# manoskary/analysisgnn

Measured on AMD Instinct MI355X. Metric: subgraph-nodes/sec fwd+bwd, HybridGNN L=3 H=256, higher is better.
Workload: dtype f32; 1 GPU; C2 (sampled, the batch a training step sees): HybridGNN L=3 H=256 out=128, 21 task heads, 32 neighbour-sampled subgraphs x (500 target notes + [5,5] hops) per GPU, per-hop counts passed (every layer trimmed); 16335 notes, 104099 edges per GPU; train step = fwd + objective (wloss) + bwd + allreduce + clip + AdamW, CSR rebuilt every step; hipGraph replay; workload_id=c2s, per_gpu_subgraphs=32, objective=wloss, parallelism=dp1, allreduce=none (one rank)

## Files before the change

analysisgnn_amd/_lib.py:

```python
from __future__ import annotations

import ctypes as C
import os
from typing import Optional, Sequence

import torch

_HERE = os.path.dirname(os.path.abspath(__file__))
LIB_PATH = os.path.join(_HERE, "libagnn_hip.so")
MAX_SEG = 32

SPMM_MEAN, SPMM_SKIP_SELF, SPMM_ACCUM = 1, 2, 4
INT32_MAX = 2 ** 31 - 1


class AgnnError(RuntimeError):
    pass


class CooSeg(C.Structure):
    _fields_ = [("row", C.c_void_p), ("col", C.c_void_p), ("etype", C.c_void_p),
                ("etype_code", C.c_int64), ("n_edges", C.c_int64), ("n_rows", C.c_int64)]


# ... 67 lines not shown
    _fields_ = [("dst", C.c_void_p), ("src", C.c_void_p * PACK_MAX_SRC), ("ld_dst", C.c_int64), ("ld_src", C.c_int64),
                ("rows", C.c_int32), ("cols", C.c_int32), ("n_src", C.c_int32), ("vec_ok", C.c_int32)]


_lib: Optional[C.CDLL] = None

SIGNATURES = {
    "agnn_last_error": (C.c_char_p, []),
    "agnn_version": (C.c_int, []),
    "agnn_csr_workspace_bytes": (C.c_size_t, [C.c_int64, C.c_int64]),
    "agnn_csr_build": (C.c_int, [C.c_int, C.POINTER(CooSeg), C.c_void_p, C.c_void_p, C.c_void_p,
                                 C.c_void_p, C.c_size_t, C.c_void_p, C.c_void_p]),
    "agnn_check_status": (C.c_int, [C.c_void_p, C.c_void_p]),
    "agnn_csr_rowend": (C.c_int, [C.c_void_p, C.c_void_p, C.c_int64, C.c_int64, C.c_void_p, C.c_void_p]),
    "agnn_csr_rowend_batch": (C.c_int, [C.c_int, C.POINTER(RowendItem), C.c_void_p]),
    "agnn_spmm_f32": (C.c_int, [C.c_int, C.POINTER(Rel), C.c_int64, C.c_int32, C.c_void_p, C.c_int64,
                                C.c_int64, C.c_void_p, C.c_int64, C.c_void_p, C.c_int32, C.c_uint32,
                                C.c_void_p]),
    "agnn_spmm_root_f32": (C.c_int, [C.c_int, C.POINTER(Rel), C.c_int64, C.c_int32, C.c_void_p, C.c_int64,
                                     C.c_int64, C.c_void_p, C.c_int64, C.c_int64, C.c_void_p, C.c_int32, C.c_uint32,
                                     C.c_void_p]),
    "agnn_gru_fwd_f32": (C.c_int, [C.c_void_p, C.c_void_p, C.c_void_p, C.c_int64, C.c_int64, C.c_int32,
                                   C.c_void_p, C.c_void_p, C.c_void_p, C.c_void_p, C.c_void_p]),
    "agnn_gru_bwd_f32": (C.c_int, [C.c_void_p, C.c_void_p, C.c_void_p, C.c_void_p, C.c_int64, C.c_int64,
                                   C.c_int32, C.c_void_p, C.c_void_p, C.c_void_p, C.c_void_p, C.c_void_p]),
    "agnn_heads_fwd_f32": (C.c_int, [C.c_void_p, C.c_int64, C.c_int64, C.c_int32, C.c_int32, C.c_int32, C.c_void_p, C.c_void_p,
                                     C.c_void_p, C.c_void_p, C.c_float, C.c_void_p, C.c_void_p, C.c_void_p, C.POINTER(C.c_int32),
                                     C.c_void_p, C.c_void_p, C.c_int64, C.c_void_p, C.c_void_p, C.c_void_p, C.c_int64, C.c_void_p]),
    "agnn_gru_hprev_f32": (C.c_int, [C.c_void_p, C.c_int64, C.c_int64, C.c_int32, C.c_void_p, C.c_void_p]),
    "agnn_hgt_attn_fwd_multi_f32": (C.c_int, [C.c_int32, C.c_void_p, C.c_int32, C.c_int32, C.c_void_p]),
    "agnn_hgt_attn_fwd_f32": (C.c_int, [C.c_int, C.POINTER(HgtRel), C.c_void_p, C.c_int64, C.c_int64, C.c_int32,
                                        C.c_int32, C.c_void_p, C.c_int64, C.c_void_p, C.c_void_p, C.c_void_p]),
    "agnn_hgt_attn_bwd_dst_f32": (C.c_int, [C.c_int, C.POINTER(HgtRel), C.c_void_p, C.c_int64, C.c_void_p, C.c_int64,
                                            C.c_void_p, C.c_int64, C.c_void_p, C.c_void_p, C.c_int64, C.c_int32,
                                            C.c_int32, C.c_void_p, C.c_int64, C.c_void_p]),
    "agnn_hgt_attn_bwd_src_batch_f32": (C.c_int, [C.c_int32, C.POINTER(HgtSrcItem), C.c_void_p, C.c_int64, C.c_void_p, C.c_int64,
                                                  C.c_int32, C.c_int32, C.c_void_p]),
    "agnn_sampler_num_nodes": (C.c_int64, [C.POINTER(Sampler)]),
    "agnn_sampler_edge_capacity": (C.c_int64, [C.POINTER(Sampler)]),
    "agnn_sample_hops": (C.c_int, [C.POINTER(Sampler), C.c_void_p]),
    "agnn_sample_members": (C.c_int, [C.c_void_p, C.c_int64, C.c_void_p, C.c_void_p, C.c_void_p, C.c_int32, C.c_int32, C.c_int32,
                                      C.POINTER(C.c_int32), C.c_int32, C.c_void_p, C.c_void_p, C.c_void_p, C.c_void_p]),
    "agnn_sample_compact_nodes": (C.c_int64, [C.POINTER(Sampler), C.POINTER(C.c_int32)]),
    "agnn_sample_compact": (C.c_int, [C.POINTER(Sampler), C.POINTER(C.c_int32), C.c_void_p, C.c_void_p, C.c_void_p]),
    "agnn_gather_rows_f32": (C.c_int, [C.c_void_p, C.c_int64, C.c_void_p, C.c_int64, C.c_int32, C.c_void_p, C.c_int64, C.c_void_p]),
    "agnn_gather_i64": (C.c_int, [C.c_void_p, C.c_int64, C.c_void_p, C.c_int64, C.c_int32, C.c_int64, C.c_void_p, C.c_int64, C.c_void_p]),
    "agnn_relt_fwd_f32": (C.c_int, [C.c_int, C.POINTER(ReltItem), C.c_int32, C.c_int32, C.c_int32, C.c_int64, C.c_void_p]),
    "agnn_relt_bwd_f32": (C.c_int, [C.c_int, C.POINTER(ReltItem), C.c_int32, C.c_int32, C.c_int32, C.c_int64, C.c_void_p]),
    "agnn_relt_dw_workspace_bytes": (C.c_size_t, [C.c_int, C.c_int32, C.c_int32, C.c_int32, C.c_int64]),
    "agnn_relt_dw_f32": (C.c_int, [C.c_int, C.POINTER(ReltItem), C.c_int32, C.c_int32, C.c_int32, C.c_int64, C.c_void_p, C.c_size_t,
                                  C.c_void_p]),
    "agnn_wgrad_batch_workspace_bytes": (C.c_size_t, [C.c_int32, C.POINTER(WgradItem)]),
    "agnn_wgrad_batch_f32": (C.c_int, [C.c_int32, C.POINTER(WgradItem), C.c_void_p, C.c_size_t, C.c_void_p]),
    "agnn_gemm_nt_f32": (C.c_int, [C.c_void_p, C.c_int64, C.c_void_p, C.c_int64, C.c_void_p, C.c_int64, C.c_int32, C.c_int32, C.c_void_p,
                                   C.c_int64, C.c_void_p]),
    "agnn_gemm_nn_f32": (C.c_int, [C.c_void_p, C.c_int64, C.c_void_p, C.c_int64, C.c_void_p, C.c_int64, C.c_int32, C.c_int32, C.c_void_p,
                                   C.c_int64, C.c_void_p]),
    "agnn_absdiff_fwd_f32": (C.c_int, [C.c_void_p, C.c_void_p, C.c_void_p, C.c_int64, C.c_int64, C.c_int32, C.c_void_p, C.c_void_p, C.c_int64,
                                       C.c_void_p]),
    "agnn_absdiff_bwd_f32": (C.c_int, [C.c_void_p, C.c_void_p, C.c_void_p, C.c_int64, C.c_int64, C.c_int32, C.c_void_p, C.c_void_p, C.c_int64,
                                       C.c_int32, C.c_int32, C.c_void_p, C.c_int64, C.c_void_p]),
    "agnn_gated_fwd_f32": (C.c_int, [C.POINTER(Gated), C.c_void_p, C.c_int64, C.c_void_p]),
    "agnn_gated_bwd_dst_f32": (C.c_int, [C.POINTER(Gated), C.c_void_p, C.c_int64, C.c_void_p, C.c_void_p, C.c_void_p]),
    "agnn_gated_bwd_src_f32": (C.c_int, [C.POINTER(Gated), C.c_void_p, C.c_int64, C.c_void_p, C.c_void_p, C.c_void_p]),
    "agnn_norm_act_workspace_bytes": (C.c_size_t, [C.c_int32]),
    "agnn_norm_act_fwd_f32": (C.c_int, [C.c_void_p, C.c_int64, C.c_void_p, C.c_void_p, C.c_int32, C.c_int64, C.c_int32, C.c_float, C.c_float,
                                        C.c_uint32, C.c_void_p, C.c_uint32, C.c_void_p, C.c_int64, C.c_void_p, C.c_void_p, C.c_void_p,
                                        C.c_void_p]),
    "agnn_norm_act_bwd_f32": (C.c_int, [C.c_void_p, C.c_int64, C.c_void_p, C.c_void_p, C.c_int32, C.c_int64, C.c_int32, C.c_float, C.c_float,
                                        C.c_uint32, C.c_void_p, C.c_uint32, C.c_void_p, C.c_int64, C.c_void_p, C.c_void_p, C.c_void_p,
                                        C.c_int64, C.c_void_p, C.c_void_p, C.c_void_p, C.c_size_t, C.c_void_p]),
    "agnn_norm_act_colsum_batch_f32": (C.c_int, [C.c_int32, C.POINTER(ColsumItem), C.c_void_p]),
    "agnn_skip_act_workspace_bytes": (C.c_size_t, []),
    "agnn_skip_act_fwd_f32": (C.c_int, [C.c_void_p, C.c_int64, C.c_void_p, C.c_int64, C.c_void_p, C.c_int64, C.c_int32, C.c_float, C.c_uint32,
                                        C.c_void_p, C.c_uint32, C.c_void_p, C.c_int64, C.c_void_p, C.c_void_p]),
    "agnn_skip_act_bwd_f32": (C.c_int, [C.c_void_p, C.c_int64, C.c_void_p, C.c_int64, C.c_void_p, C.c_int64, C.c_int32, C.c_float, C.c_uint32,
                                        C.c_void_p, C.c_uint32, C.c_void_p, C.c_int64, C.c_void_p, C.c_int64, C.c_void_p, C.c_int64, C.c_void_p,
                                        C.c_void_p, C.c_size_t, C.c_void_p]),
    "agnn_norm_act_colsum_f32": (C.c_int, [C.c_void_p, C.c_size_t, C.c_int64, C.c_int32, C.c_void_p, C.c_void_p, C.c_void_p]),
    "agnn_wgrad_workspace_bytes": (C.c_size_t, [C.c_int64, C.c_int32, C.c_int32]),
    "agnn_wgrad_f32": (C.c_int, [C.c_void_p, C.c_int64, C.c_void_p, C.c_int64, C.c_int64, C.c_int32, C.c_int32, C.c_void_p,
                                 C.c_int64, C.c_void_p, C.c_void_p, C.c_size_t, C.c_void_p]),
    "agnn_pack_f32": (C.c_int, [C.c_int32, C.POINTER(PackItem), C.c_void_p]),
    "agnn_debug_stamp": (C.c_int, [C.c_void_p, C.c_void_p]),
    "agnn_gproj_fwd_f32": (C.c_int, [C.c_void_p, C.c_int64, C.c_void_p, C.c_void_p, C.c_void_p, C.c_int32, C.c_int32, C.c_int32,
                                     C.c_int64, C.c_void_p, C.c_int64, C.c_void_p]),
    "agnn_gproj_workspace_bytes": (C.c_size_t, [C.c_int64, C.c_int32, C.c_int32, C.c_int32]),
    "agnn_gproj_bwd_f32": (C.c_int, [C.c_void_p, C.c_int64, C.c_void_p, C.c_int64, C.c_void_p, C.c_void_p, C.c_int32, C.c_int32,
                                     C.c_int32, C.c_int32, C.c_int64, C.c_void_p, C.c_int64, C.c_void_p, C.c_void_p, C.c_void_p,
                                     C.c_size_t, C.c_void_p]),
    "agnn_spmm_self_grad_f32": (C.c_int, [C.c_void_p, C.c_int64, C.c_int64, C.c_int32, C.c_void_p, C.c_int64, C.c_int64, C.c_int32,
                                          C.c_void_p, C.c_int64, C.c_int32, C.c_void_p]),
    "agnn_embed_cat_fwd_f32": (C.c_int, [C.c_void_p, C.c_int64, C.c_int32, C.c_int64, C.c_int32, C.POINTER(C.c_void_p),
                                         C.POINTER(C.c_void_p), C.POINTER(C.c_int32), C.c_int32, C.c_void_p, C.c_int64, C.c_void_p]),
    "agnn_embed_workspace_bytes": (C.c_size_t, [C.c_int32, C.POINTER(C.c_int32), C.c_int32]),
    "agnn_embed_cat_bwd_f32": (C.c_int, [C.c_void_p, C.c_int64, C.c_int32, C.c_int64, C.c_int32, C.POINTER(C.c_void_p),
                                         C.POINTER(C.c_int32), C.c_int32, C.c_void_p, C.c_void_p, C.c_size_t, C.c_void_p]),
    "agnn_train_loss_workspace_bytes": (C.c_size_t, []),
    "agnn_train_loss_f32": (C.c_int, [C.c_void_p, C.c_int64, C.c_void_p, C.c_int32, C.c_void_p, C.c_int64, C.c_float, C.c_int64,
                                      C.c_void_p, C.c_int64, C.c_int32, C.c_float, C.c_void_p, C.c_float, C.c_void_p, C.c_void_p,
                                      C.c_void_p, C.c_void_p, C.c_void_p, C.c_void_p, C.c_void_p, C.c_void_p, C.c_size_t,
                                      C.c_void_p]),
    "agnn_train_loss_final_f32": (C.c_int, [C.c_void_p, C.c_int64, C.c_void_p, C.c_int32, C.c_void_p, C.c_int64, C.c_float, C.c_int64,
                                            C.c_void_p, C.c_int64, C.c_int32, C.c_float, C.c_void_p, C.c_float, C.c_void_p, C.c_void_p,
                                            C.c_void_p, C.c_void_p, C.c_void_p, C.c_void_p, C.c_void_p, C.c_void_p, C.c_int64, C.c_void_p,
                                            C.c_size_t, C.c_void_p]),
# ... 116 lines not shown
```

analysisgnn_amd/csrc/embed.hip:

```cpp
#include <cstdlib>

#include "agnn_common.h"

namespace {

constexpr int kMaxTab = AGNN_EMBED_MAX_TABLES;
constexpr int kSlices = 128;

struct EmbFwd {
  const float* x;
  int64_t ld_x;
  int32_t in_x, n_tab, dim;
  int64_t n_rows;
  const int64_t* idx[kMaxTab];
  const float* tab[kMaxTab];
  int32_t vocab[kMaxTab];
  float* out;
  int64_t ld_out;
};

__global__ __launch_bounds__(256) void k_embed_cat_fwd(EmbFwd a) {
  const int64_t total = a.n_rows * a.ld_out;
  for (int64_t e = static_cast<int64_t>(blockIdx.x) * 256 + threadIdx.x; e < total; e += static_cast<int64_t>(gridDim.x) * 256) {
    const int64_t row = e / a.ld_out;
    const int col = static_cast<int>(e - row * a.ld_out);
    float v = 0.f;
    if (col < a.in_x) {
      v = a.x[row * a.ld_x + col];
    } else {
      const int c = col - a.in_x;
      const int t = c / a.dim;
      if (t < a.n_tab) {
        int64_t id = a.idx[t][row];
        id = id < 0 ? 0 : (id >= a.vocab[t] ? a.vocab[t] - 1 : id);
        v = a.tab[t][id * a.dim + (c - t * a.dim)];
      }
    }
    a.out[e] = v;
  }
}

struct EmbBwd {
  const float* dout;
  int64_t ld_dout;
  int32_t col0, n_tab, dim, dim_pad, v_total, v_pad;
  int64_t n_rows;
  const int64_t* idx[kMaxTab];
  int32_t vbase[kMaxTab + 1];
  float* slab;
};

__global__ __launch_bounds__(256) void k_embed_bwd(EmbBwd a) {
  const int lane = threadIdx.x & 63;
  const int wave = __builtin_amdgcn_readfirstlane(threadIdx.x >> 6);
  const int vg = blockIdx.x;
  int t = 0;
  while (t + 1 < a.n_tab && vg >= a.vbase[t + 1]) ++t;
  const int64_t v = vg - a.vbase[t];
  const int64_t* idx = a.idx[t];
  const int col_base = a.col0 + t * a.dim;
  const int part = blockIdx.y * 4 + wave;
  const int64_t per = ((a.n_rows + kSlices * 4 - 1) / (kSlices * 4) + 63) & ~int64_t{63};
  const int64_t r0 = part * per;
  int64_t r1 = r0 + per;
  if (r1 > a.n_rows) r1 = a.n_rows;
  float* dst = a.slab + (static_cast<int64_t>(part) * a.v_pad + vg) * a.dim_pad;
  for (int c0 = 0; c0 < a.dim; c0 += 64) {
    const bool on = c0 + lane < a.dim;
    float acc = 0.f;
    for (int64_t base = r0; base < r1; base += 64) {
      const int64_t r = base + lane;
      const bool hit = r < r1 && idx[r] == v;
      uint64_t m = __ballot(hit);
      while (m) {
        const int b = __builtin_ctzll(m);
        m &= m - 1;
        if (on) acc += a.dout[(base + b) * a.ld_dout + col_base + c0 + lane];
      }
    }
    if (on) dst[c0 + lane] = acc;
  }
}

constexpr int kEmbLdsFloats = 4096;

template <int NCG>
__global__ __launch_bounds__(256) void k_embed_bwd_rows(EmbBwd a) {
  __shared__ float s_acc[4][kEmbLdsFloats];
  const int lane = threadIdx.x & 63;
  const int wave = __builtin_amdgcn_readfirstlane(threadIdx.x >> 6);
  float* acc = s_acc[wave];
  const int img = a.v_total * a.dim;
  for (int e = lane; e < img; e += 64) acc[e] = 0.f;
  const int part = blockIdx.x * 4 + wave;
  const int64_t per = (a.n_rows + kSlices * 4 - 1) / (kSlices * 4);
  const int64_t r0 = part * per;
  int64_t r1 = r0 + per;
  if (r1 > a.n_rows) r1 = a.n_rows;
  const int width = a.n_tab * a.dim;
  bool on[NCG];
  int cc[NCG], vb[NCG], vn[NCG], col[NCG];
  const int64_t* idx[NCG];
#pragma unroll
  for (int g = 0; g < NCG; ++g) {
    const int c = 64 * g + lane;
    on[g] = c < width;
    const int t = on[g] ? c / a.dim : 0;
    cc[g] = c - t * a.dim;
    idx[g] = a.idx[t];
    vb[g] = a.vbase[t];
    vn[g] = a.vbase[t + 1] - vb[g];
    col[g] = a.col0 + (on[g] ? c : 0);
  }
  __builtin_amdgcn_fence(__ATOMIC_RELEASE, "wavefront");
  __builtin_amdgcn_wave_barrier();
  constexpr int RB = NCG <= 2 ? 8 : 4;
  for (int64_t base = r0; base < r1; base += RB) {
    float val[RB][NCG];
    int64_t id[RB][NCG];
#pragma unroll
    for (int u = 0; u < RB; ++u) {
      const int64_t r = base + u < r1 ? base + u : r1 - 1;
#pragma unroll
      for (int g = 0; g < NCG; ++g) {
        id[u][g] = idx[g][r];
        val[u][g] = a.dout[r * a.ld_dout + col[g]];
      }
    }
#pragma unroll
    for (int u = 0; u < RB; ++u)
#pragma unroll
      for (int g = 0; g < NCG; ++g)
        if (on[g] && base + u < r1 && id[u][g] >= 0 && id[u][g] < vn[g]) acc[(vb[g] + static_cast<int>(id[u][g])) * a.dim + cc[g]] += val[u][g];
  }
  __builtin_amdgcn_fence(__ATOMIC_RELEASE, "wavefront");
  __builtin_amdgcn_wave_barrier();
  float* dst = a.slab + static_cast<int64_t>(part) * a.v_pad * a.dim_pad;
  for (int e = lane; e < img; e += 64) dst[e] = acc[e];
}

}

extern "C" size_t agnn_embed_workspace_bytes(int32_t n_tab, const int32_t* vocab, int32_t dim) {
  if (n_tab <= 0 || n_tab > kMaxTab || !vocab || dim <= 0) return 0;
  int64_t v_total = 0;
  for (int t = 0; t < n_tab; ++t) v_total += vocab[t];
  return static_cast<size_t>(kSlices * 4) * static_cast<size_t>(v_total) * static_cast<size_t>((dim + 1) & ~1) * sizeof(float) + 256;
}

extern "C" int agnn_embed_cat_fwd_f32(const float* x, int64_t ld_x, int32_t in_x, int64_t n_rows, int32_t n_tab,
                                      const int64_t* const* idx, const float* const* tables, const int32_t* vocab,
                                      int32_t dim, float* out, int64_t ld_out, agnn_stream_t stream_) {
  using namespace agnn;
  if (n_tab < 0 || n_tab > kMaxTab) return fail(AGNN_EINVAL, "embed_cat: n_tab=%d not in [0,%d]", n_tab, kMaxTab);
  if (n_rows < 0 || in_x < 0 || dim <= 0) return fail(AGNN_EINVAL, "embed_cat: bad sizes n_rows=%lld in_x=%d dim=%d", (long long)n_rows, in_x, dim);
  if (ld_out < static_cast<int64_t>(in_x) + static_cast<int64_t>(n_tab) * dim || (in_x > 0 && ld_x < in_x))
    return fail(AGNN_EINVAL, "embed_cat: leading dimension smaller than the row");
  if (n_rows == 0) return AGNN_OK;
  if (!out || (in_x > 0 && !x) || (n_tab > 0 && (!idx || !tables || !vocab))) return fail(AGNN_EINVAL, "embed_cat: null argument");
  EmbFwd a{};
  a.x = x; a.ld_x = ld_x; a.in_x = in_x; a.n_tab = n_tab; a.dim = dim; a.n_rows = n_rows; a.out = out; a.ld_out = ld_out;
  for (int t = 0; t < n_tab; ++t) {
    if (!idx[t] || !tables[t] || vocab[t] <= 0) return fail(AGNN_EINVAL, "embed_cat: table %d: null pointer or empty table", t);
    a.idx[t] = idx[t]; a.tab[t] = tables[t]; a.vocab[t] = vocab[t];
  }
  const int64_t total = n_rows * ld_out;
  int64_t blocks = (total + 255) / 256;
  if (blocks > 8192) blocks = 8192;
  hipLaunchKernelGGL(k_embed_cat_fwd, dim3(static_cast<unsigned>(blocks)), dim3(256), 0, static_cast<hipStream_t>(stream_), a);
  return check_launch("embed_cat_fwd");
}

extern "C" int agnn_embed_cat_bwd_f32(const float* dout, int64_t ld_dout, int32_t col0, int64_t n_rows, int32_t n_tab,
                                      const int64_t* const* idx, const int32_t* vocab, int32_t dim, float* dtables,
                                      void* workspace, size_t workspace_bytes, agnn_stream_t stream_) {
  using namespace agnn;
  if (n_tab <= 0 || n_tab > kMaxTab) return fail(AGNN_EINVAL, "embed_bwd: n_tab=%d not in [1,%d]", n_tab, kMaxTab);
  if (n_rows < 0 || col0 < 0 || dim <= 0 || (dim & 1)) return fail(AGNN_EINVAL, "embed_bwd: bad sizes n_rows=%lld col0=%d dim=%d (dim must be even)", (long long)n_rows, col0, dim);
  if (!dout || !idx || !vocab || !dtables || !workspace) return fail(AGNN_EINVAL, "embed_bwd: null argument");
  if (ld_dout < static_cast<int64_t>(col0) + static_cast<int64_t>(n_tab) * dim) return fail(AGNN_EINVAL, "embed_bwd: ld_dout smaller than the row");
  if (reinterpret_cast<uintptr_t>(dtables) & 7u) return fail(AGNN_EALIGN, "embed_bwd: dtables must be 8-byte aligned");
  const size_t need = agnn_embed_workspace_bytes(n_tab, vocab, dim);
  if (need == 0 || workspace_bytes < need) return fail(AGNN_ENOMEM, "embed_bwd: workspace %zu < %zu bytes", workspace_bytes, need);
  EmbBwd a{};
  a.dout = dout; a.ld_dout = ld_dout; a.col0 = col0; a.n_tab = n_tab; a.dim = dim; a.dim_pad = dim; a.n_rows = n_rows;
  int vt = 0;
  for (int t = 0; t < n_tab; ++t) {
    if (!idx[t] || vocab[t] <= 0) return fail(AGNN_EINVAL, "embed_bwd: table %d: null index pointer or empty table", t);
    a.idx[t] = idx[t];
    a.vbase[t] = vt;
    vt += vocab[t];
  }
  a.vbase[n_tab] = vt;
  a.v_total = vt; a.v_pad = vt;
  a.slab = reinterpret_cast<float*>((reinterpret_cast<uintptr_t>(workspace) + 255) & ~uintptr_t{255});
  hipStream_t s = static_cast<hipStream_t>(stream_);
  const int ncg = (n_tab * dim + 63) / 64;
  if (static_cast<int64_t>(vt) * dim <= kEmbLdsFloats && ncg <= 4) {
    if (ncg == 1) hipLaunchKernelGGL(k_embed_bwd_rows<1>, dim3(kSlices), dim3(256), 0, s, a);
    else if (ncg == 2) hipLaunchKernelGGL(k_embed_bwd_rows<2>, dim3(kSlices), dim3(256), 0, s, a);
    else if (ncg == 3) hipLaunchKernelGGL(k_embed_bwd_rows<3>, dim3(kSlices), dim3(256), 0, s, a);
    else hipLaunchKernelGGL(k_embed_bwd_rows<4>, dim3(kSlices), dim3(256), 0, s, a);
    if (int rc = check_launch("embed_bwd(rows)")) return rc;
  } else {
    hipLaunchKernelGGL(k_embed_bwd, dim3(vt, kSlices), dim3(256), 0, s, a);
    if (int rc = check_launch("embed_bwd")) return rc;
  }
  return launch_slab_reduce(a.slab, nullptr, kSlices * 4, vt, dim, vt, dim, dtables, dim, nullptr, s);
}
```

analysisgnn_amd/csrc/wgrad.hip:

```cpp
#include "agnn_common.h"

namespace {

typedef float f32x16 __attribute__((ext_vector_type(16)));

struct WgArgs {
  const float* dy;
  const float* x;
  int64_t ld_dy, ld_x;
  int32_t n, out_f, in_f;
  int32_t rows_per_slice;
  int32_t tiles_in;
  float* slab;
  float* slab_b;
  int32_t out_pad, in_pad;
};

__device__ __forceinline__ void wgrad_tile(const WgArgs& a, const int tile, const int slice) {
  const int lane = threadIdx.x & 63;
  const int wave = threadIdx.x >> 6;
  const int wm = wave >> 1, wn = wave & 1;
  const int to = tile / a.tiles_in, ti = tile - to * a.tiles_in;
  const int kk = lane >> 5, c32 = lane & 31;
  const int ocol = to * 128 + wm * 64 + 2 * c32;
// ... 77 lines not shown
  }
  for (; c + 3 <= nfull; c += 3) {
    fetch(c + 2, a2, b2);
    mma(a0, b0);
    fetch(c + 3, a0, b0);
    mma(a1, b1);
    fetch(c + 4, a1, b1);
    mma(a2, b2);
  }
  fetch(c + 2, a2, b2);
  if (c < nchunks) mma_tail(c, a0, b0);
  if (c + 1 < nchunks) mma_tail(c + 1, a1, b1);
  if (c + 2 < nchunks) mma_tail(c + 2, a2, b2);
  float* slab = a.slab + (static_cast<int64_t>(slice) * a.out_pad) * a.in_pad;
  const int ob = to * 128 + wm * 64, ib = ti * 128 + wn * 64;
#pragma unroll
  for (int r = 0; r < 16; ++r) {
    const int i = (r & 3) + 8 * (r >> 2) + 4 * kk;
    float* row0 = slab + static_cast<int64_t>(ob + 2 * i) * a.in_pad + ib + 2 * c32;
    float* row1 = row0 + a.in_pad;
    *reinterpret_cast<float2*>(row0) = make_float2(acc00[r], acc01[r]);
    *reinterpret_cast<float2*>(row1) = make_float2(acc10[r], acc11[r]);
  }
  if (a.slab_b != nullptr && wn == 0) {
    bs0 += __shfl_xor(bs0, 32, 64);
    bs1 += __shfl_xor(bs1, 32, 64);
    if (kk == 0 && ti == 0)
      *reinterpret_cast<float2*>(a.slab_b + static_cast<int64_t>(slice) * a.out_pad + ocol) = make_float2(bs0, bs1);
  }
}

__global__ __launch_bounds__(256) void k_wgrad(WgArgs a) { wgrad_tile(a, blockIdx.x, blockIdx.y); }

constexpr int kWgBatchMax = 16;

struct WgBatch {
  WgArgs it[kWgBatchMax];
  int32_t first[kWgBatchMax + 1];
  int32_t tiles[kWgBatchMax];
  int32_t n;
};

__global__ __launch_bounds__(256) void k_wgrad_batch(WgBatch b) {
  int i = 0;
  const int blk = blockIdx.x;
  while (i + 1 < b.n && blk >= b.first[i + 1]) ++i;
  const int local = blk - b.first[i];
  const int tiles = b.tiles[i];
  const int slice = local / tiles;
  wgrad_tile(b.it[i], local - slice * tiles, slice);
}


__device__ __forceinline__ void wgrad_reduce_blocks(const float* __restrict__ slab, const float* __restrict__ slab_b, int S, int out_f, int in_f,
                                                    int out_pad, int in_pad, float* __restrict__ dw, int64_t ld_dw, float* __restrict__ db,
                                                    const int block, const int n_blocks) {
  __shared__ float2 part[8][32];
  const int col = threadIdx.x & 31, sg = threadIdx.x >> 5;
  const int half_in = in_f >> 1;
  const int64_t total = static_cast<int64_t>(out_f) * half_in;
  const int64_t plane = static_cast<int64_t>(out_pad) * in_pad;
  for (int64_t e0 = static_cast<int64_t>(block) * 32; e0 < total; e0 += static_cast<int64_t>(n_blocks) * 32) {
    const int64_t e = e0 + col;
    float2 s = make_float2(0.f, 0.f);
    int o = 0, i = 0;
    if (e < total) {
      o = static_cast<int>(e / half_in);
      i = static_cast<int>(e - static_cast<int64_t>(o) * half_in) * 2;
      const float* p = slab + static_cast<int64_t>(o) * in_pad + i;
      for (int k = sg; k < S; k += 8) {
        const float2 v = *reinterpret_cast<const float2*>(p + k * plane);
        s.x += v.x;
        s.y += v.y;
      }
    }
    part[sg][col] = s;
    __syncthreads();
    if (sg == 0 && e < total) {
      float2 t = part[0][col];
#pragma unroll
      for (int g = 1; g < 8; ++g) { t.x += part[g][col].x; t.y += part[g][col].y; }
      *reinterpret_cast<float2*>(dw + static_cast<int64_t>(o) * ld_dw + i) = t;
    }
    __syncthreads();
  }
  if (db != nullptr) {
    __shared__ float partb[8][32];
    for (int e0 = block * 32; e0 < out_f; e0 += n_blocks * 32) {
      const int e = e0 + col;
      float s = 0.f;
      if (e < out_f)
        for (int k = sg; k < S; k += 8) s += slab_b[static_cast<int64_t>(k) * out_pad + e];
      partb[sg][col] = s;
      __syncthreads();
      if (sg == 0 && e < out_f) {
        float t = partb[0][col];
#pragma unroll
        for (int g = 1; g < 8; ++g) t += partb[g][col];
        db[e] = t;
      }
      __syncthreads();
    }
  }
}

__global__ __launch_bounds__(256) void k_wgrad_reduce(const float* __restrict__ slab, const float* __restrict__ slab_b, int S,
                                                      int out_f, int in_f, int out_pad, int in_pad, float* __restrict__ dw,
                                                      int64_t ld_dw, float* __restrict__ db) {
  wgrad_reduce_blocks(slab, slab_b, S, out_f, in_f, out_pad, in_pad, dw, ld_dw, db, blockIdx.x, gridDim.x);
}

struct RedItem {
  const float* slab;
  const float* slab_b;
  float* dw;
  float* db;
  int64_t ld_dw;
  int32_t S, out_f, in_f, out_pad, in_pad;
};
struct RedBatch {
  RedItem it[kWgBatchMax];
  int32_t first[kWgBatchMax + 1];
  int32_t n;
};

__global__ __launch_bounds__(256) void k_wgrad_reduce_batch(RedBatch b) {
  int i = 0;
  const int blk = blockIdx.x;
  while (i + 1 < b.n && blk >= b.first[i + 1]) ++i;
  const RedItem& r = b.it[i];
  wgrad_reduce_blocks(r.slab, r.slab_b, r.S, r.out_f, r.in_f, r.out_pad, r.in_pad, r.dw, r.ld_dw, r.db, blk - b.first[i], b.first[i + 1] - b.first[i]);
}

struct Plan {
  int tiles_out, tiles_in, S, rows_per_slice, out_pad, in_pad;
};

Plan make_plan(int64_t n, int out_f, int in_f) {
  Plan p;
  p.tiles_out = (out_f + 127) / 128;
  p.tiles_in = (in_f + 127) / 128;
  p.out_pad = p.tiles_out * 128;
  p.in_pad = p.tiles_in * 128;
  const int tiles = p.tiles_out * p.tiles_in;
  int64_t S = 512 / tiles;
  const int64_t max_s = (n + 63) / 64;
  if (S > max_s) S = max_s;
  if (S > 64) S = 64;
  if (S < 1) S = 1;
  int64_t rps = (n + S - 1) / S;
  rps = (rps + 1) & ~int64_t{1};
  p.rows_per_slice = static_cast<int>(rps);
  p.S = static_cast<int>((n + rps - 1) / rps);
  return p;
}

}

int agnn::launch_slab_reduce(const float* slab, const float* slab_b, int S, int out_f, int in_f, int out_pad, int in_pad,
                             float* dw, int64_t ld_dw, float* db, hipStream_t s) {
  const int64_t total = static_cast<int64_t>(out_f) * (in_f >> 1);
  int blocks = static_cast<int>((total + 31) / 32);
  if (blocks > 4096) blocks = 4096;
  if (blocks < 1) blocks = 1;
  hipLaunchKernelGGL(k_wgrad_reduce, dim3(blocks), dim3(256), 0, s, slab, slab_b, S, out_f, in_f, out_pad, in_pad, dw, ld_dw, db);
  return check_launch("slab_reduce");
}

extern "C" size_t agnn_wgrad_workspace_bytes(int64_t n, int32_t out_f, int32_t in_f) {
  if (n <= 0 || out_f <= 0 || in_f <= 0) return 0;
  const Plan p = make_plan(n, out_f, in_f);
  return (static_cast<size_t>(p.S) * p.out_pad * p.in_pad + static_cast<size_t>(p.S) * p.out_pad) * sizeof(float) + 256;
}

extern "C" int agnn_wgrad_f32(const float* dy, int64_t ld_dy, const float* x, int64_t ld_x, int64_t n, int32_t out_f,
                              int32_t in_f, float* dw, int64_t ld_dw, float* db, void* workspace, size_t workspace_bytes,
                              agnn_stream_t stream_) {
  using namespace agnn;
  if (n <= 0 || n >= (int64_t{1} << 31) || out_f <= 0 || in_f <= 0) return fail(AGNN_EINVAL, "wgrad: bad sizes n=%lld out=%d in=%d", (long long)n, out_f, in_f);
  if ((out_f & 1) || (in_f & 1) || (ld_dy & 1) || (ld_x & 1) || (ld_dw & 1)) return fail(AGNN_EALIGN, "wgrad: widths and leading dimensions must be even");
  if (!dy || !x || !dw || !workspace) return fail(AGNN_EINVAL, "wgrad: null argument");
  if ((reinterpret_cast<uintptr_t>(dy) | reinterpret_cast<uintptr_t>(x) | reinterpret_cast<uintptr_t>(dw) | reinterpret_cast<uintptr_t>(db)) & 7u)
    return fail(AGNN_EALIGN, "wgrad: pointers must be 8-byte aligned");
  if (ld_dy < out_f || ld_x < in_f || ld_dw < in_f) return fail(AGNN_EINVAL, "wgrad: leading dimension smaller than the width");
  const size_t need = agnn_wgrad_workspace_bytes(n, out_f, in_f);
  if (workspace_bytes < need) return fail(AGNN_ENOMEM, "wgrad: workspace %zu < %zu bytes", workspace_bytes, need);
  const Plan p = make_plan(n, out_f, in_f);
  if ((static_cast<int64_t>(p.rows_per_slice) + 128) * (ld_dy > ld_x ? ld_dy : ld_x) * 4 >= (int64_t{1} << 32))
    return fail(AGNN_EINVAL, "wgrad: a row slice (%d rows x ld) exceeds the kernel's 32-bit byte offsets", p.rows_per_slice);
  char* ws = reinterpret_cast<char*>((reinterpret_cast<uintptr_t>(workspace) + 255) & ~uintptr_t{255});
  float* slab = reinterpret_cast<float*>(ws);
  float* slab_b = slab + static_cast<size_t>(p.S) * p.out_pad * p.in_pad;
  WgArgs a{dy, x, ld_dy, ld_x, static_cast<int32_t>(n), out_f, in_f, p.rows_per_slice, p.tiles_in, slab,
           db ? slab_b : nullptr, p.out_pad, p.in_pad};
  hipStream_t s = static_cast<hipStream_t>(stream_);
  hipLaunchKernelGGL(k_wgrad, dim3(p.tiles_out * p.tiles_in, p.S), dim3(256), 0, s, a);
  if (int rc = check_launch("wgrad")) return rc;
  return launch_slab_reduce(slab, db ? slab_b : nullptr, p.S, out_f, in_f, p.out_pad, p.in_pad, dw, ld_dw, db, s);
}

namespace {
struct BatchPlan {
  int n;
  int tiles_out[kWgBatchMax], tiles_in[kWgBatchMax], S[kWgBatchMax], rps[kWgBatchMax];
  size_t slab_off[kWgBatchMax], slabb_off[kWgBatchMax], total_floats;
};

int batch_plan(int n_items, const agnn_wgrad_item_t* items, BatchPlan& bp) {
  using namespace agnn;
  if (n_items <= 0 || n_items > kWgBatchMax || !items) return fail(AGNN_EINVAL, "wgrad_batch: %d items (1 .. %d)", n_items, kWgBatchMax);
  bp.n = n_items;
  int64_t tiles = 0;
  for (int i = 0; i < n_items; ++i) {
    const agnn_wgrad_item_t& it = items[i];
    if (it.n <= 0 || it.n >= (int64_t{1} << 31) || it.out_f <= 0 || it.in_f <= 0) return fail(AGNN_EINVAL, "wgrad_batch: item %d: bad sizes", i);
    bp.tiles_out[i] = (it.out_f + 127) / 128;
    bp.tiles_in[i] = (it.in_f + 127) / 128;
    tiles += static_cast<int64_t>(bp.tiles_out[i]) * bp.tiles_in[i];
  }
// ... 74 lines not shown
```

include/agnn.h:

```cpp
#ifndef AGNN_H_
#define AGNN_H_

#include <stddef.h>
#include <stdint.h>

#ifdef __cplusplus
extern "C" {
#endif

typedef void* agnn_stream_t;

#define AGNN_OK        0
#define AGNN_EINVAL  (-22)
#define AGNN_EALIGN  (-14)
#define AGNN_ENOMEM  (-12)
#define AGNN_ERUNTIME (-5)

#define AGNN_MAX_SEG 32

const char* agnn_last_error(void);
int agnn_version(void);

typedef struct {
  const int64_t* row;
// ... 145 lines not shown
                         float* out_s, float* out_d, int64_t ld_out, agnn_stream_t stream);
int agnn_absdiff_bwd_f32(const int32_t* rowptr, const int32_t* col, const float* h, int64_t ld, int64_t n_rows, int32_t H,
                         const float* gd, const float* gs, int64_t ld_g, int32_t by_col, int32_t accumulate, float* out,
                         int64_t ld_out, agnn_stream_t stream);

#define AGNN_NA_PRE_RELU  1u
#define AGNN_NA_POST_RELU 2u
size_t agnn_norm_act_workspace_bytes(int32_t H);
int agnn_norm_act_fwd_f32(const float* x, int64_t ld_x, const float* gamma, const float* beta, int32_t seg,
                          int64_t n, int32_t H, float eps, float p, uint32_t flags, const int64_t* rng_state, uint32_t call_id, float* y,
                          int64_t ld_y, float* mean, float* rstd, int64_t* rng_used, agnn_stream_t stream);
int agnn_norm_act_bwd_f32(const float* x, int64_t ld_x, const float* gamma, const float* beta, int32_t seg,
                          int64_t n, int32_t H, float eps, float p, uint32_t flags, const int64_t* rng_state, uint32_t call_id,
                          const float* dy, int64_t ld_dy, const float* mean, const float* rstd, float* dx,
                          int64_t ld_dx, float* dgamma, float* dbeta, void* workspace, size_t workspace_bytes,
                          agnn_stream_t stream);

typedef struct {
  const void* workspace;
  size_t workspace_bytes;
  int64_t n;
  int32_t H;
  float* dgamma;
  float* dbeta;
} agnn_colsum_item_t;
int agnn_norm_act_colsum_batch_f32(int32_t n_items, const agnn_colsum_item_t* items , agnn_stream_t stream);

size_t agnn_skip_act_workspace_bytes(void);
int agnn_skip_act_fwd_f32(const float* x, int64_t ld_x, const float* o, int64_t ld_o, const float* skip, int64_t n, int32_t H, float p,
                          uint32_t flags, const int64_t* rng_state, uint32_t call_id, float* z, int64_t ld_z, int64_t* rng_used,
                          agnn_stream_t stream);
int agnn_skip_act_bwd_f32(const float* x, int64_t ld_x, const float* o, int64_t ld_o, const float* skip, int64_t n, int32_t H, float p,
                          uint32_t flags, const int64_t* rng_state, uint32_t call_id, const float* dz, int64_t ld_dz, float* dx,
                          int64_t ld_dx, float* dout, int64_t ld_do, float* dskip, void* workspace, size_t workspace_bytes,
                          agnn_stream_t stream);
int agnn_norm_act_colsum_f32(const void* workspace, size_t workspace_bytes, int64_t n, int32_t H, float* dgamma, float* dbeta,
                             agnn_stream_t stream);

size_t agnn_wgrad_workspace_bytes(int64_t n, int32_t out_f, int32_t in_f);
int agnn_wgrad_f32(const float* dy, int64_t ld_dy, const float* x, int64_t ld_x, int64_t n, int32_t out_f,
                   int32_t in_f, float* dw, int64_t ld_dw, float* db, void* workspace, size_t workspace_bytes,
                   agnn_stream_t stream);
typedef struct {
  const float* dy;
  const float* x;
  float* dw;
  float* db;
  int64_t ld_dy, ld_x, ld_dw, n;
  int32_t out_f, in_f;
} agnn_wgrad_item_t;
size_t agnn_wgrad_batch_workspace_bytes(int32_t n_items, const agnn_wgrad_item_t* items );
int agnn_wgrad_batch_f32(int32_t n_items, const agnn_wgrad_item_t* items , void* workspace, size_t workspace_bytes,
                         agnn_stream_t stream);

#define AGNN_PACK_MAX_SRC   8
#define AGNN_PACK_MAX_ITEMS 24
typedef struct {
  float* dst;
  const float* src[AGNN_PACK_MAX_SRC];
  int64_t ld_dst, ld_src;
  int32_t rows, cols, n_src, vec_ok;
} agnn_pack_item_t;
int agnn_pack_f32(int32_t n_items, const agnn_pack_item_t* items , agnn_stream_t stream);

int agnn_debug_stamp(uint64_t* slot , agnn_stream_t stream);

#define AGNN_EMBED_MAX_TABLES 4
int agnn_embed_cat_fwd_f32(const float* x, int64_t ld_x, int32_t in_x, int64_t n_rows, int32_t n_tab,
                           const int64_t* const* idx, const float* const* tables, const int32_t* vocab, int32_t dim,
                           float* out, int64_t ld_out, agnn_stream_t stream);
size_t agnn_embed_workspace_bytes(int32_t n_tab, const int32_t* vocab, int32_t dim);
int agnn_embed_cat_bwd_f32(const float* dout, int64_t ld_dout, int32_t col0, int64_t n_rows, int32_t n_tab,
                           const int64_t* const* idx, const int32_t* vocab, int32_t dim, float* dtables,
                           void* workspace, size_t workspace_bytes, agnn_stream_t stream);

int agnn_heads_fwd_f32(const float* x, int64_t ld_x, int64_t n_rows, int32_t in_f, int32_t hidden, int32_t T, const float* w1,
                       const float* b1, const float* gamma, const float* beta, float eps, const float* w2, const float* b2,
                       const int32_t* offs_dev, const int32_t* offs_host, float* z, float* y, int64_t ld_h, float* mean,
                       float* rstd, float* logits, int64_t ld_o, agnn_stream_t stream);

int agnn_gproj_fwd_f32(const float* a, int64_t ld_a, const float* w, const float* b, const int32_t* seg_off,
                       int32_t n_groups, int32_t K, int32_t n_tiles32, int64_t n_rows, float* out, int64_t ld_out,
                       agnn_stream_t stream);
size_t agnn_gproj_workspace_bytes(int64_t n_rows, int32_t sum_c, int32_t K, int32_t n_tiles32);
int agnn_gproj_bwd_f32(const float* dout, int64_t ld_dout, const float* a, int64_t ld_a, const float* w,
                       const int32_t* seg_off, int32_t n_groups, int32_t K, int32_t n_tiles32, int32_t sum_c,
                       int64_t n_rows, float* da, int64_t ld_da, float* dw, float* db, void* workspace,
                       size_t workspace_bytes, agnn_stream_t stream);

int agnn_multitask_ce_f32(const float* logits, int64_t ld, const int32_t* seg_off, int32_t n_tasks,
                          const int64_t* labels, int64_t n_rows, float label_smoothing,
                          int64_t ignore_index, float* row_loss, float* dlogits, float* loss, float* inv_count,
                          agnn_stream_t stream);
int agnn_multitask_ce_scale_f32(const float* dlogits, int64_t ld, const int32_t* seg_off, int32_t n_tasks,
                                int64_t n_rows, int32_t n_cols, const float* scale, float* out, int64_t ld_out,
                                agnn_stream_t stream);

size_t agnn_train_loss_workspace_bytes(void);
int agnn_train_loss_f32(const float* logits, int64_t ld, const int32_t* seg_off, int32_t n_tasks, const int64_t* labels,
                        int64_t n_rows, float label_smoothing, int64_t ignore_index, const float* feat, int64_t ld_feat,
                        int32_t feat_cols, float lambda_feat, const float* task_param, float ce_scale, float* row_loss,
                        float* dlogits, float* loss, float* inv_count, float* total, float* wscale, float* dparam,
                        void* workspace, size_t workspace_bytes, agnn_stream_t stream);
int agnn_train_loss_final_f32(const float* logits, int64_t ld, const int32_t* seg_off, int32_t n_tasks, const int64_t* labels,
                              int64_t n_rows, float label_smoothing, int64_t ignore_index, const float* feat, int64_t ld_feat,
                              int32_t feat_cols, float lambda_feat, const float* task_param, float ce_scale, float* row_loss,
// ... 67 lines not shown
```

Measured before the change: 5.581 million subgraph-nodes/s.

## Rework embedding fwd/bwd kernels and slab reduction for small workloads

The embedding-concat forward now gives each row to one wave and loads the table indices once per row, with an optional float4 store path, instead of running a flat per-element grid-stride loop. The embedding backward removes the LDS row-accumulator kernel and always uses the per-vocab kernel. That kernel now builds an LDS list of matching rows in 512-row chunks and reads 16 rows at a time to keep more loads in flight, with fewer slices (16 instead of 128). The slab reduction kernel picks 64-thread blocks for small outputs and stages its loads 8 deep. A new exported slab_sum entry point is added. The per-vocab backward may do redundant index scans compared with the removed LDS path when the vocabulary is large.

```diff
diff --git a/analysisgnn_amd/_lib.py b/analysisgnn_amd/_lib.py
--- a/analysisgnn_amd/_lib.py
+++ b/analysisgnn_amd/_lib.py
@@ -143,6 +143,8 @@
                                   C.c_void_p]),
     "agnn_wgrad_batch_workspace_bytes": (C.c_size_t, [C.c_int32, C.POINTER(WgradItem)]),
     "agnn_wgrad_batch_f32": (C.c_int, [C.c_int32, C.POINTER(WgradItem), C.c_void_p, C.c_size_t, C.c_void_p]),
+    "agnn_slab_sum_f32": (C.c_int, [C.c_void_p, C.c_void_p, C.c_int32, C.c_int32, C.c_int32, C.c_int32, C.c_int32, C.c_void_p, C.c_int64,
+                                    C.c_void_p, C.c_void_p]),
     "agnn_gemm_nt_f32": (C.c_int, [C.c_void_p, C.c_int64, C.c_void_p, C.c_int64, C.c_void_p, C.c_int64, C.c_int32, C.c_int32, C.c_void_p,
                                    C.c_int64, C.c_void_p]),
     "agnn_gemm_nn_f32": (C.c_int, [C.c_void_p, C.c_int64, C.c_void_p, C.c_int64, C.c_void_p, C.c_int64, C.c_int32, C.c_int32, C.c_void_p,
diff --git a/analysisgnn_amd/csrc/embed.hip b/analysisgnn_amd/csrc/embed.hip
--- a/analysisgnn_amd/csrc/embed.hip
+++ b/analysisgnn_amd/csrc/embed.hip
@@ -5,7 +5,9 @@
 namespace {
 
 constexpr int kMaxTab = AGNN_EMBED_MAX_TABLES;
-constexpr int kSlices = 128;
+constexpr int kSlices = 16;
+constexpr int kChunk = 512;
+constexpr int kRowsInFlight = 16;
 
 struct EmbFwd {
   const float* x;
@@ -19,24 +21,44 @@
   int64_t ld_out;
 };
 
+__device__ __forceinline__ float embed_cat_value(const EmbFwd& a, int64_t row, int col, const int64_t (&id)[kMaxTab]) {
+  if (col < a.in_x) return a.x[row * a.ld_x + col];
+  const int c = col - a.in_x;
+  const int t = c / a.dim;
+  float v = 0.f;
+#pragma unroll
+  for (int u = 0; u < kMaxTab; ++u)
+    if (u == t && u < a.n_tab) v = a.tab[u][id[u] * a.dim + (c - u * a.dim)];
+  return v;
+}
+
+template <bool VEC4>
 __global__ __launch_bounds__(256) void k_embed_cat_fwd(EmbFwd a) {
-  const int64_t total = a.n_rows * a.ld_out;
-  for (int64_t e = static_cast<int64_t>(blockIdx.x) * 256 + threadIdx.x; e < total; e += static_cast<int64_t>(gridDim.x) * 256) {
-    const int64_t row = e / a.ld_out;
-    const int col = static_cast<int>(e - row * a.ld_out);
-    float v = 0.f;
-    if (col < a.in_x) {
-      v = a.x[row * a.ld_x + col];
-    } else {
-      const int c = col - a.in_x;
-      const int t = c / a.dim;
-      if (t < a.n_tab) {
-        int64_t id = a.idx[t][row];
-        id = id < 0 ? 0 : (id >= a.vocab[t] ? a.vocab[t] - 1 : id);
-        v = a.tab[t][id * a.dim + (c - t * a.dim)];
-      }
+  const int lane = threadIdx.x & 63;
+  const int64_t row = static_cast<int64_t>(blockIdx.x) * 4 + (threadIdx.x >> 6);
+  if (row >= a.n_rows) return;
+  int64_t id[kMaxTab];
+#pragma unroll
+  for (int u = 0; u < kMaxTab; ++u) {
+    id[u] = 0;
+    if (u < a.n_tab) {
+      const int64_t i = a.idx[u][row];
+      id[u] = i < 0 ? 0 : (i >= a.vocab[u] ? a.vocab[u] - 1 : i);
     }
-    a.out[e] = v;
+  }
+  float* dst = a.out + row * a.ld_out;
+  const int ld = static_cast<int>(a.ld_out);
+  if (VEC4) {
+    for (int c0 = lane * 4; c0 < ld; c0 += 256) {
+      float4 v;
+      v.x = embed_cat_value(a, row, c0, id);
+      v.y = embed_cat_value(a, row, c0 + 1, id);
+      v.z = embed_cat_value(a, row, c0 + 2, id);
+      v.w = embed_cat_value(a, row, c0 + 3, id);
+      *reinterpret_cast<float4*>(dst + c0) = v;
+    }
+  } else {
+    for (int c = lane; c < ld; c += 64) dst[c] = embed_cat_value(a, row, c, id);
   }
 }
 
@@ -51,8 +73,10 @@
 };
 
 __global__ __launch_bounds__(256) void k_embed_bwd(EmbBwd a) {
+  __shared__ int s_rows[4][kChunk];
   const int lane = threadIdx.x & 63;
   const int wave = __builtin_amdgcn_readfirstlane(threadIdx.x >> 6);
+  int* list = s_rows[wave];
   const int vg = blockIdx.x;
   int t = 0;
   while (t + 1 < a.n_tab && vg >= a.vbase[t + 1]) ++t;
@@ -60,83 +84,53 @@
   const int64_t* idx = a.idx[t];
   const int col_base = a.col0 + t * a.dim;
   const int part = blockIdx.y * 4 + wave;
-  const int64_t per = ((a.n_rows + kSlices * 4 - 1) / (kSlices * 4) + 63) & ~int64_t{63};
+  const int64_t per = (a.n_rows + kSlices * 4 - 1) / (kSlices * 4);
   const int64_t r0 = part * per;
   int64_t r1 = r0 + per;
   if (r1 > a.n_rows) r1 = a.n_rows;
   float* dst = a.slab + (static_cast<int64_t>(part) * a.v_pad + vg) * a.dim_pad;
   for (int c0 = 0; c0 < a.dim; c0 += 64) {
     const bool on = c0 + lane < a.dim;
+    const float* src = a.dout + col_base + (on ? c0 + lane : 0);
     float acc = 0.f;
-    for (int64_t base = r0; base < r1; base += 64) {
-      const int64_t r = base + lane;
-      const bool hit = r < r1 && idx[r] == v;
-      uint64_t m = __ballot(hit);
-      while (m) {
-        const int b = __builtin_ctzll(m);
-        m &= m - 1;
-        if (on) acc += a.dout[(base + b) * a.ld_dout + col_base + c0 + lane];
+    for (int64_t base = r0; base < r1; base += kChunk) {
+      int64_t id[kChunk / 64];
+#pragma unroll
+      for (int u = 0; u < kChunk / 64; ++u) {
+        const int64_t r = base + 64 * u + lane;
+        id[u] = idx[r < r1 ? r : r1 - 1];
       }
+      int n = 0;
+#pragma unroll
+      for (int u = 0; u < kChunk / 64; ++u) {
+        const bool hit = base + 64 * u + lane < r1 && id[u] == v;
+        const uint64_t m = __ballot(hit);
+        const int before = __builtin_amdgcn_mbcnt_hi(static_cast<uint32_t>(m >> 32), __builtin_amdgcn_mbcnt_lo(static_cast<uint32_t>(m), 0u));
+        if (hit) list[n + before] = 64 * u + lane;
+        n += __popcll(m);
+      }
+      __builtin_amdgcn_fence(__ATOMIC_RELEASE, "wavefront");
+      __builtin_amdgcn_wave_barrier();
+      for (int j0 = 0; j0 < n; j0 += 64) {
+        const int m = n - j0 < 64 ? n - j0 : 64;
+        const int mine = list[j0 + (lane < m ? lane : m - 1)];
+        for (int j = 0; j < m; j += kRowsInFlight) {
+          float val[kRowsInFlight];
+#pragma unroll
+          for (int u = 0; u < kRowsInFlight; ++u) {
+            const int off = __builtin_amdgcn_readlane(mine, j + u < m ? j + u : m - 1);
+            val[u] = src[(base + off) * a.ld_dout];
+          }
+#pragma unroll
+          for (int u = 0; u < kRowsInFlight; ++u)
+            if (j + u < m) acc += val[u];
+        }
+      }
+      __builtin_amdgcn_fence(__ATOMIC_RELEASE, "wavefront");
+      __builtin_amdgcn_wave_barrier();
     }
     if (on) dst[c0 + lane] = acc;
   }
-}
-
-constexpr int kEmbLdsFloats = 4096;
-
-template <int NCG>
-__global__ __launch_bounds__(256) void k_embed_bwd_rows(EmbBwd a) {
-  __shared__ float s_acc[4][kEmbLdsFloats];
-  const int lane = threadIdx.x & 63;
-  const int wave = __builtin_amdgcn_readfirstlane(threadIdx.x >> 6);
-  float* acc = s_acc[wave];
-  const int img = a.v_total * a.dim;
-  for (int e = lane; e < img; e += 64) acc[e] = 0.f;
-  const int part = blockIdx.x * 4 + wave;
-  const int64_t per = (a.n_rows + kSlices * 4 - 1) / (kSlices * 4);
-  const int64_t r0 = part * per;
-  int64_t r1 = r0 + per;
-  if (r1 > a.n_rows) r1 = a.n_rows;
-  const int width = a.n_tab * a.dim;
-  bool on[NCG];
-  int cc[NCG], vb[NCG], vn[NCG], col[NCG];
-  const int64_t* idx[NCG];
-#pragma unroll
-  for (int g = 0; g < NCG; ++g) {
-    const int c = 64 * g + lane;
-    on[g] = c < width;
-    const int t = on[g] ? c / a.dim : 0;
-    cc[g] = c - t * a.dim;
-    idx[g] = a.idx[t];
-    vb[g] = a.vbase[t];
-    vn[g] = a.vbase[t + 1] - vb[g];
-    col[g] = a.col0 + (on[g] ? c : 0);
-  }
-  __builtin_amdgcn_fence(__ATOMIC_RELEASE, "wavefront");
-  __builtin_amdgcn_wave_barrier();
-  constexpr int RB = NCG <= 2 ? 8 : 4;
-  for (int64_t base = r0; base < r1; base += RB) {
-    float val[RB][NCG];
-    int64_t id[RB][NCG];
-#pragma unroll
-    for (int u = 0; u < RB; ++u) {
-      const int64_t r = base + u < r1 ? base + u : r1 - 1;
-#pragma unroll
-      for (int g = 0; g < NCG; ++g) {
-        id[u][g] = idx[g][r];
-        val[u][g] = a.dout[r * a.ld_dout + col[g]];
-      }
-    }
-#pragma unroll
-    for (int u = 0; u < RB; ++u)
-#pragma unroll
-      for (int g = 0; g < NCG; ++g)
-        if (on[g] && base + u < r1 && id[u][g] >= 0 && id[u][g] < vn[g]) acc[(vb[g] + static_cast<int>(id[u][g])) * a.dim + cc[g]] += val[u][g];
-  }
-  __builtin_amdgcn_fence(__ATOMIC_RELEASE, "wavefront");
-  __builtin_amdgcn_wave_barrier();
-  float* dst = a.slab + static_cast<int64_t>(part) * a.v_pad * a.dim_pad;
-  for (int e = lane; e < img; e += 64) dst[e] = acc[e];
 }
 
 }
@@ -164,10 +158,11 @@
     if (!idx[t] || !tables[t] || vocab[t] <= 0) return fail(AGNN_EINVAL, "embed_cat: table %d: null pointer or empty table", t);
     a.idx[t] = idx[t]; a.tab[t] = tables[t]; a.vocab[t] = vocab[t];
   }
-  const int64_t total = n_rows * ld_out;
-  int64_t blocks = (total + 255) / 256;
-  if (blocks > 8192) blocks = 8192;
-  hipLaunchKernelGGL(k_embed_cat_fwd, dim3(static_cast<unsigned>(blocks)), dim3(256), 0, static_cast<hipStream_t>(stream_), a);
+  if (ld_out >= (int64_t{1} << 31) || (n_rows + 3) / 4 >= (int64_t{1} << 31)) return fail(AGNN_EINVAL, "embed_cat: n_rows or ld_out too large");
+  const dim3 grid(static_cast<unsigned>((n_rows + 3) / 4));
+  hipStream_t s = static_cast<hipStream_t>(stream_);
+  if ((ld_out & 3) == 0 && (reinterpret_cast<uintptr_t>(out) & 15u) == 0) hipLaunchKernelGGL(k_embed_cat_fwd<true>, grid, dim3(256), 0, s, a);
+  else hipLaunchKernelGGL(k_embed_cat_fwd<false>, grid, dim3(256), 0, s, a);
   return check_launch("embed_cat_fwd");
 }
 
@@ -195,16 +190,7 @@
   a.v_total = vt; a.v_pad = vt;
   a.slab = reinterpret_cast<float*>((reinterpret_cast<uintptr_t>(workspace) + 255) & ~uintptr_t{255});
   hipStream_t s = static_cast<hipStream_t>(stream_);
-  const int ncg = (n_tab * dim + 63) / 64;
-  if (static_cast<int64_t>(vt) * dim <= kEmbLdsFloats && ncg <= 4) {
-    if (ncg == 1) hipLaunchKernelGGL(k_embed_bwd_rows<1>, dim3(kSlices), dim3(256), 0, s, a);
-    else if (ncg == 2) hipLaunchKernelGGL(k_embed_bwd_rows<2>, dim3(kSlices), dim3(256), 0, s, a);
-    else if (ncg == 3) hipLaunchKernelGGL(k_embed_bwd_rows<3>, dim3(kSlices), dim3(256), 0, s, a);
-    else hipLaunchKernelGGL(k_embed_bwd_rows<4>, dim3(kSlices), dim3(256), 0, s, a);
-    if (int rc = check_launch("embed_bwd(rows)")) return rc;
-  } else {
-    hipLaunchKernelGGL(k_embed_bwd, dim3(vt, kSlices), dim3(256), 0, s, a);
-    if (int rc = check_launch("embed_bwd")) return rc;
-  }
+  hipLaunchKernelGGL(k_embed_bwd, dim3(vt, kSlices), dim3(256), 0, s, a);
+  if (int rc = check_launch("embed_bwd")) return rc;
   return launch_slab_reduce(a.slab, nullptr, kSlices * 4, vt, dim, vt, dim, dtables, dim, nullptr, s);
 }
diff --git a/analysisgnn_amd/csrc/wgrad.hip b/analysisgnn_amd/csrc/wgrad.hip
--- a/analysisgnn_amd/csrc/wgrad.hip
+++ b/analysisgnn_amd/csrc/wgrad.hip
@@ -153,26 +153,38 @@
 }
 
 
+constexpr int kRedStage = 8;
+
 __device__ __forceinline__ void wgrad_reduce_blocks(const float* __restrict__ slab, const float* __restrict__ slab_b, int S, int out_f, int in_f,
                                                     int out_pad, int in_pad, float* __restrict__ dw, int64_t ld_dw, float* __restrict__ db,
                                                     const int block, const int n_blocks) {
   __shared__ float2 part[8][32];
-  const int col = threadIdx.x & 31, sg = threadIdx.x >> 5;
+  const int shift = blockDim.x == 256 ? 5 : 3;
+  const int ncol = 1 << shift;
+  const int col = threadIdx.x & (ncol - 1), sg = threadIdx.x >> shift;
+  const int cnt = S > sg ? (S - sg + 7) >> 3 : 0;
   const int half_in = in_f >> 1;
   const int64_t total = static_cast<int64_t>(out_f) * half_in;
   const int64_t plane = static_cast<int64_t>(out_pad) * in_pad;
-  for (int64_t e0 = static_cast<int64_t>(block) * 32; e0 < total; e0 += static_cast<int64_t>(n_blocks) * 32) {
+  for (int64_t e0 = static_cast<int64_t>(block) * ncol; e0 < total; e0 += static_cast<int64_t>(n_blocks) * ncol) {
     const int64_t e = e0 + col;
     float2 s = make_float2(0.f, 0.f);
     int o = 0, i = 0;
     if (e < total) {
       o = static_cast<int>(e / half_in);
       i = static_cast<int>(e - static_cast<int64_t>(o) * half_in) * 2;
-      const float* p = slab + static_cast<int64_t>(o) * in_pad + i;
-      for (int k = sg; k < S; k += 8) {
-        const float2 v = *reinterpret_cast<const float2*>(p + k * plane);
-        s.x += v.x;
-        s.y += v.y;
+      const float* p = slab + static_cast<int64_t>(o) * in_pad + i + sg * plane;
+      for (int j0 = 0; j0 < cnt; j0 += kRedStage) {
+        float2 v[kRedStage];
+#pragma unroll
+        for (int u = 0; u < kRedStage; ++u)
+          if (j0 + u < cnt) v[u] = *reinterpret_cast<const float2*>(p + static_cast<int64_t>(j0 + u) * 8 * plane);
+#pragma unroll
+        for (int u = 0; u < kRedStage; ++u)
+          if (j0 + u < cnt) {
+            s.x += v[u].x;
+            s.y += v[u].y;
+          }
       }
     }
     part[sg][col] = s;
@@ -187,11 +199,21 @@
   }
   if (db != nullptr) {
     __shared__ float partb[8][32];
-    for (int e0 = block * 32; e0 < out_f; e0 += n_blocks * 32) {
+    for (int e0 = block * ncol; e0 < out_f; e0 += n_blocks * ncol) {
       const int e = e0 + col;
       float s = 0.f;
-      if (e < out_f)
-        for (int k = sg; k < S; k += 8) s += slab_b[static_cast<int64_t>(k) * out_pad + e];
+      if (e < out_f) {
+        const float* p = slab_b + static_cast<int64_t>(sg) * out_pad + e;
+        for (int j0 = 0; j0 < cnt; j0 += kRedStage) {
+          float v[kRedStage];
+#pragma unroll
+          for (int u = 0; u < kRedStage; ++u)
+            if (j0 + u < cnt) v[u] = p[static_cast<int64_t>(j0 + u) * 8 * out_pad];
+#pragma unroll
+          for (int u = 0; u < kRedStage; ++u)
+            if (j0 + u < cnt) s += v[u];
+        }
+      }
       partb[sg][col] = s;
       __syncthreads();
       if (sg == 0 && e < out_f) {
@@ -261,11 +283,23 @@
 int agnn::launch_slab_reduce(const float* slab, const float* slab_b, int S, int out_f, int in_f, int out_pad, int in_pad,
                              float* dw, int64_t ld_dw, float* db, hipStream_t s) {
   const int64_t total = static_cast<int64_t>(out_f) * (in_f >> 1);
-  int blocks = static_cast<int>((total + 31) / 32);
+  const int threads = total < 32 * 256 ? 64 : 256;
+  int blocks = static_cast<int>((total + threads / 8 - 1) / (threads / 8));
   if (blocks > 4096) blocks = 4096;
   if (blocks < 1) blocks = 1;
-  hipLaunchKernelGGL(k_wgrad_reduce, dim3(blocks), dim3(256), 0, s, slab, slab_b, S, out_f, in_f, out_pad, in_pad, dw, ld_dw, db);
+  hipLaunchKernelGGL(k_wgrad_reduce, dim3(blocks), dim3(threads), 0, s, slab, slab_b, S, out_f, in_f, out_pad, in_pad, dw, ld_dw, db);
   return check_launch("slab_reduce");
+}
+
+extern "C" int agnn_slab_sum_f32(const float* slab, const float* slab_b, int32_t S, int32_t out_f, int32_t in_f, int32_t out_pad, int32_t in_pad,
+                                 float* dw, int64_t ld_dw, float* db, agnn_stream_t stream_) {
+  using namespace agnn;
+  if (S <= 0 || out_f <= 0 || in_f <= 0 || out_pad < out_f || in_pad < in_f) return fail(AGNN_EINVAL, "slab_sum: bad sizes S=%d out=%d in=%d pads=%d,%d", S, out_f, in_f, out_pad, in_pad);
+  if ((in_f & 1) || (in_pad & 1) || (ld_dw & 1)) return fail(AGNN_EALIGN, "slab_sum: in_f, in_pad and ld_dw must be even");
+  if (!slab || !dw || (db != nullptr) != (slab_b != nullptr)) return fail(AGNN_EINVAL, "slab_sum: null argument (slab_b and db go together)");
+  if (ld_dw < in_f) return fail(AGNN_EINVAL, "slab_sum: ld_dw smaller than the width");
+  if ((reinterpret_cast<uintptr_t>(slab) | reinterpret_cast<uintptr_t>(dw)) & 7u) return fail(AGNN_EALIGN, "slab_sum: pointers must be 8-byte aligned");
+  return launch_slab_reduce(slab, slab_b, S, out_f, in_f, out_pad, in_pad, dw, ld_dw, db, static_cast<hipStream_t>(stream_));
 }
 
 extern "C" size_t agnn_wgrad_workspace_bytes(int64_t n, int32_t out_f, int32_t in_f) {
diff --git a/include/agnn.h b/include/agnn.h
--- a/include/agnn.h
+++ b/include/agnn.h
@@ -221,6 +221,8 @@
 size_t agnn_wgrad_batch_workspace_bytes(int32_t n_items, const agnn_wgrad_item_t* items );
 int agnn_wgrad_batch_f32(int32_t n_items, const agnn_wgrad_item_t* items , void* workspace, size_t workspace_bytes,
                          agnn_stream_t stream);
+int agnn_slab_sum_f32(const float* slab, const float* slab_b, int32_t S, int32_t out_f, int32_t in_f, int32_t out_pad, int32_t in_pad,
+                      float* dw, int64_t ld_dw, float* db, agnn_stream_t stream);
 
 #define AGNN_PACK_MAX_SRC   8
 #define AGNN_PACK_MAX_ITEMS 24
```

New measurement: 5.615 million subgraph-nodes/s (median of 6 runs). Within noise of the previous version (+0.6%).
